# Patrick-McKeever/P2P-DHTs

Hardware: AMD Instinct MI355X
Metric: successor lookups/sec (whole node) + % HBM roofline, 2^24-peer ring, 1/2/4/8 GPUs (higher is better)
Workload: dtype u128; 1 GPU; C4 finger-routed lookups with hop counts (per GPU): 2^24-peer ring, 2^25 keys/GPU/step, src = q mod N, splitmix seeds 0x5EED0005/0x5EED0006; peers=16777216, keys_per_gpu=33554432, global_batch=33554432

## Files before the change

### p2p-dhts_amd/chordx/ring.py

```python
from __future__ import annotations

import ctypes

import numpy as np

from . import _lib as L

try:
    import torch
except Exception:
    torch = None


def _is_dev(x) -> bool:
    return torch is not None and isinstance(x, torch.Tensor) and x.is_cuda


def _keys_np(a) -> np.ndarray:
    return np.ascontiguousarray(np.asarray(a, dtype=np.uint64).reshape(-1, 2))


def _check_dev(t, esize: int, name: str, device=None, count=None):
    if not _is_dev(t):
        return
# ... 174 lines not shown
            sl = self._prep_u32(succs, "succs", self.n)
            ns = 1 if sl.ndim == 1 else int(sl.shape[1])
        arrs = [a for a in (al, sl) if a is not None]
        mk = self._mem(*arrs) if arrs else L.CX_MEM_HOST
        L.check(L.lib().cx_liveness_upload(self._h, _ptr(al), _ptr(sl), int(ns), int(rule), mk))

    def fingers_device(self):
        p = ctypes.c_void_p()
        L.check(L.lib().cx_fingers_device(self._h, ctypes.byref(p)))
        if not p.value:
            return None
        return _wrap_device(p.value, (self.n, L.CX_FINGERS), torch.int32, self.device, self)

    def set_route_variant(self, v: int):
        f = L.lib().cxi_set_route_variant
        f.argtypes = [ctypes.c_void_p, ctypes.c_int]
        L.check(f(self._h, v))

    def route_info(self):
        f = L.lib().cxi_route_info
        f.argtypes = [ctypes.c_void_p, ctypes.POINTER(ctypes.c_int),
                      ctypes.POINTER(ctypes.c_uint64), ctypes.POINTER(ctypes.c_uint64)]
        v, e, b = ctypes.c_int(), ctypes.c_uint64(), ctypes.c_uint64()
        L.check(f(self._h, ctypes.byref(v), ctypes.byref(e), ctypes.byref(b)))
        return v.value, e.value, b.value

    def route_counters(self, enable: bool):
        f = L.lib().cxi_route_counters
        f.argtypes = [ctypes.c_void_p, ctypes.c_int, ctypes.c_void_p]
        out = np.zeros(4, dtype=np.uint64)
        L.check(f(self._h, int(bool(enable)), _ptr(out)))
        return None if enable else tuple(int(x) for x in out)

    def gather_probe(self, lanes: int = 1 << 19, hops: int = 64, span: int = 0) -> float:
        if span:
            f = L.lib().cxi_gather_probe_span
            f.argtypes = [ctypes.c_void_p, ctypes.c_int, ctypes.c_int, ctypes.c_uint64,
                          ctypes.POINTER(ctypes.c_double)]
            r = ctypes.c_double()
            L.check(f(self._h, lanes, hops, span, ctypes.byref(r)))
            return r.value
        f = L.lib().cxi_gather_probe
        f.argtypes = [ctypes.c_void_p, ctypes.c_int, ctypes.c_int,
                      ctypes.POINTER(ctypes.c_double)]
        r = ctypes.c_double()
        L.check(f(self._h, lanes, hops, ctypes.byref(r)))
        return r.value

    def route_table_hash(self, arc: bool = False) -> int:
        f = L.lib().cxi_route_table_hash
        f.argtypes = [ctypes.c_void_p, ctypes.c_int, ctypes.POINTER(ctypes.c_uint64)]
        h = ctypes.c_uint64()
        L.check(f(self._h, int(bool(arc)), ctypes.byref(h)))
        return h.value

    def set_table_build(self, v: int):
        f = L.lib().cxi_set_table_build
        f.argtypes = [ctypes.c_void_p, ctypes.c_int]
        L.check(f(self._h, v))

    def set_route_depth(self, R: int):
        f = L.lib().cxi_set_route_depth
        f.argtypes = [ctypes.c_void_p, ctypes.c_int]
        L.check(f(self._h, int(R)))

    def set_fingers_repair(self, on: bool):
# ... 397 lines not shown
```

### p2p-dhts_amd/csrc/cx_api.hip

```cpp
#include <hip/hip_runtime.h>

#include <cstdio>
#include <cstdlib>
#include <cstring>
#include <initializer_list>
#include <algorithm>
#include <atomic>
#include <memory>
#include <mutex>
#include <string>
#include <vector>

#include "cx_kernels.hpp"

namespace {

thread_local std::string g_err;

int fail(int code, const std::string &msg) {
    g_err = msg;
    return code;
}

#define CX_HIP(expr)                                                                      \
// ... 311 lines not shown
    size_t n = 0;
    cell128 *d_ring = nullptr;
    size_t ring_cap = 0;
    cell128 *d_eyt = nullptr;
    uint32_t *d_fingers = nullptr;
    bool fingers_converged = false;
    std::atomic<bool> rows_deferred{false};
    std::mutex rows_mu;
    std::shared_ptr<PlaneSet> planes;
    std::shared_ptr<PlaneSet> parent_planes;
    int fingers_repair = 0;
    int planes_repaired = 0;
    uint64_t repair_searched = 0;
    cell128 *d_ring_ext = nullptr;
    int rt_l0 = 128, rt_R = 0;
    int depth_override = 0;
    uint64_t *d_tree = nullptr;
    bool tree_valid = false;
    int pk_ib = 1;
    uint64_t *d_cz = nullptr;
    int table_build = 0;
    bool cz_valid = false;
    uint64_t cz_escapes = 0;
    int route_variant = -1;
    cell128 *d_min_keys = nullptr;
    uint32_t *d_preds = nullptr;
    uint8_t *d_alive = nullptr;
    uint32_t *d_succs = nullptr;
    int succ_ns = 0;
    int fwd_rule = CX_FWD_CHORD;
    bool liveness = false;
    uint32_t *d_scratch = nullptr;
    unsigned long long *d_stats = nullptr;
    bool counting = false;
    uint64_t *d_arc_tree = nullptr;
    ArcBound *d_arc_bounds = nullptr;
    int arc_world = 0, arc_rank = -1, arc_Lh = 128, arc_nb = 0;
    uint32_t arc_plo = 0, arc_M = 0;
    size_t arc_bytes = 0;

    uint4 *d_dir = nullptr;
    uint32_t *d_ring_key = nullptr;
    int dir_k = 1;
    int search_variant = 1;
    void *d_sltab = nullptr;
    int sl_b = 0, sl_steps = 0;
    bool sl_dev16 = false;
    std::mutex sl_mu;
    std::atomic<bool> sl_ready{false};
    cell128 *d_stree = nullptr;
    uint32_t *d_eyt_rank = nullptr;
    int churn_variant = 1;
    uint64_t serial = 0;
    uint64_t churn_parent = 0;
    uint32_t *d_o2n_canon = nullptr;
    size_t o2n_canon_n = 0;
    uint4 *d_cdir = nullptr;
    int cdir_kb = 0;
    size_t cdir_bytes = 0;
    int misplaced_variant = 1;

    EytView eyt() const {
        EytView v;
        v.E = d_eyt;
        v.n = (uint32_t)n;
        v.h = 63 - __builtin_clzll((unsigned long long)n);
// ... 52 lines not shown
}

template <class T>
int stage_out(T *dst, size_t count, int memkind, DBuf &tmp, T **dev, hipStream_t s) {
    if (count == 0) {
        *dev = dst;
        return CX_OK;
    }
    CX_CHECK(dst != nullptr, CX_E_INVALID, "null output buffer");
    if (memkind == CX_MEM_DEVICE) {
        *dev = dst;
        return CX_OK;
    }
    CX_CHECK(memkind == CX_MEM_HOST, CX_E_INVALID, "bad memkind");
    CX_HIP(tmp.alloc_stage(count * sizeof(T), s));
    *dev = tmp.as<T>();
    return CX_OK;
}

template <class T>
int finish_out(T *dst, const T *dev, size_t count, int memkind, hipStream_t s) {
    if (memkind == CX_MEM_HOST && count) {
        CX_HIP(hipMemcpyAsync(dst, dev, count * sizeof(T), hipMemcpyDeviceToHost, s));
        CX_HIP(hipStreamSynchronize(s));
    }
    return CX_OK;
}

int sync_if_host(int memkind, hipStream_t s) {
    if (memkind == CX_MEM_HOST) CX_HIP(hipStreamSynchronize(s));
    return CX_OK;
}

struct RingRes {
    int device;
    hipStream_t stream;
    void *scratch;
};
std::mutex g_res_mu;
std::vector<RingRes> g_res;
constexpr size_t RES_KEEP = 16;

int alloc_ring(int device, cx_ring **out) {
    cx_ring *r = new cx_ring();
    r->device = device;
    {
        std::lock_guard<std::mutex> g(g_res_mu);
        for (size_t k = g_res.size(); k-- > 0;)
            if (g_res[k].device == device) {
                r->own_stream = g_res[k].stream;
                r->d_scratch = static_cast<uint32_t *>(g_res[k].scratch);
                g_res.erase(g_res.begin() + k);
                break;
            }
    }
    if (!r->own_stream) {
        hipError_t e = hipStreamCreateWithFlags(&r->own_stream, hipStreamNonBlocking);
        if (e != hipSuccess) {
            delete r;
            return fail(CX_E_HIP, std::string("hipStreamCreate: ") + hipGetErrorString(e));
        }
        e = dev_malloc(&r->d_scratch, 1024);
        if (e != hipSuccess) {
            (void)hipStreamDestroy(r->own_stream);
            delete r;
            return fail(CX_E_HIP, std::string("hipMalloc: ") + hipGetErrorString(e));
        }
    }
    r->stream = r->own_stream;
    static std::atomic<uint64_t> next_serial{1};
    r->serial = next_serial++;
    *out = r;
    return CX_OK;
}

void free_ring(cx_ring *r) {
    if (!r) return;
    (void)hipSetDevice(r->device);
    if (r->stream) (void)hipStreamSynchronize(r->stream);
    if (r->own_stream) (void)hipStreamSynchronize(r->own_stream);
    r->planes.reset();
    r->parent_planes.reset();
    table_free(r->device, r->d_ring, r->ring_cap * sizeof(cell128));
    (void)hipFree(r->d_eyt);
    table_free(r->device, r->d_dir, r->d_dir ? ((size_t)1 << r->dir_k) * sizeof(uint4) : 0);
    table_free(r->device, r->d_ring_key, r->n * sizeof(uint32_t));
    const size_t ent = r->n * (size_t)r->rt_R;
    table_free(r->device, r->d_fingers, r->n * CX_FINGERS * sizeof(uint32_t));
    table_free(r->device, r->d_tree, ent * 64);
    table_free(r->device, r->d_cz, ent * 128);
    (void)hipFree(r->d_stree);
    (void)hipFree(r->d_eyt_rank);
    (void)hipFree(r->d_sltab);
    table_free(r->device, r->d_ring_ext, (r->n + 1) * sizeof(cell128));
    (void)hipFree(r->d_min_keys);
    (void)hipFree(r->d_preds);
    (void)hipFree(r->d_alive);
    (void)hipFree(r->d_succs);
    table_free(r->device, r->d_arc_tree, r->arc_bytes);
// ... 807 lines not shown

int cx_route(const cx_ring *ring, const uint32_t *src, const cx_u128 *keys, size_t q,
             uint32_t *owner, uint8_t *hops, uint8_t *status, int memkind) {
    CX_CHECK(ring != nullptr, CX_E_INVALID, "null ring");
    CX_CHECK(ring->d_fingers != nullptr || ring->rows_deferred, CX_E_STATE,
             "finger table not built (cx_fingers_build / cx_fingers_upload)");
    int rc = use_device(ring);
    if (rc) return rc;
    hipStream_t s = ring->stream;
    DBuf ts, tk, to, th, tst;
    const uint32_t *dsrc;
    const cx_u128 *dk;
    uint32_t *dow;
    uint8_t *dh, *dst = nullptr;
    if ((rc = stage_in(src, q, memkind, ts, &dsrc, s))) return rc;
    if ((rc = stage_in(keys, q, memkind, tk, &dk, s))) return rc;
    if ((rc = stage_out(owner, q, memkind, to, &dow, s))) return rc;
    if ((rc = stage_out(hops, q, memkind, th, &dh, s))) return rc;
    if (status && (rc = stage_out(status, q, memkind, tst, &dst, s))) return rc;
    if (!ring->literal()) {
        int e2 = ensure_route_table(const_cast<cx_ring *>(ring), s);
        if (e2) return e2;
    }
    const int v = ring->literal() ? -1 : ring->variant();
    if (v != 5 || !ring->cz_valid) {
        int e2 = ensure_fingers_rows(const_cast<cx_ring *>(ring), s);
        if (e2) return e2;
    }
    SearchView dsv = ring->sv();
    dsv.dir = ring->d_dir;
    if (v == 5 && ring->cz_valid)
        CX_HIP(cxk::route_walk(ring->d_ring_ext, ring->d_ring, ring->n, ring->d_cz, ring->rt_l0,
                               ring->pk_ib, dsv, dsrc, reinterpret_cast<const cell128 *>(dk), q,
                               dow, dh, dst, ring->counting ? ring->d_stats : nullptr, s));
    else if (v == 4 && ring->tree_valid)
        CX_HIP(cxk::route_tree(ring->d_ring_ext, ring->d_ring, ring->n, ring->d_tree, ring->rt_l0,
                               ring->rt_R, ring->pk_ib, ring->d_fingers, dsrc,
                               reinterpret_cast<const cell128 *>(dk), q, dow, dh, dst, s));
    else
        CX_HIP(cxk::route(ring->d_ring, ring->n, ring->d_fingers, ring->d_min_keys,
                          ring->d_preds, ring->lit(), ring->literal(), dsrc,
                          reinterpret_cast<const cell128 *>(dk), q, dow, dh, dst, s));
    if (memkind == CX_MEM_HOST && q) {
        CX_HIP(hipMemcpyAsync(owner, dow, q * sizeof(uint32_t), hipMemcpyDeviceToHost, s));
        CX_HIP(hipMemcpyAsync(hops, dh, q, hipMemcpyDeviceToHost, s));
        if (status) CX_HIP(hipMemcpyAsync(status, dst, q, hipMemcpyDeviceToHost, s));
        CX_HIP(hipStreamSynchronize(s));
    }
    return CX_OK;
}

int cx_nsucc(const cx_ring *ring, const cx_u128 *keys, size_t q, int n, uint32_t *lists,
             uint8_t *count, int memkind) {
    CX_CHECK(ring != nullptr, CX_E_INVALID, "null ring");
    CX_CHECK(n >= 1 && n <= CX_MAX_NSUCC, CX_E_INVALID, "n must be in [1, 16]");
    int rc = use_device(ring);
    if (rc) return rc;
    hipStream_t s = ring->stream;
    DBuf tk, tl, tc;
    const cx_u128 *dk;
    uint32_t *dl;
    uint8_t *dc;
    if ((rc = stage_in(keys, q, memkind, tk, &dk, s))) return rc;
    if ((rc = stage_out(lists, q * (size_t)n, memkind, tl, &dl, s))) return rc;
    if ((rc = stage_out(count, q, memkind, tc, &dc, s))) return rc;
    CX_HIP(cxk::nsucc(ring->sv(), reinterpret_cast<const cell128 *>(dk), q, n, dl, dc, s));
    if (memkind == CX_MEM_HOST && q) {
// ... 982 lines not shown
    CX_CHECK(variant == -1 || variant == 0 || variant == 4 || variant == 5, CX_E_INVALID,
             "variant must be -1 (auto), 0, 4 or 5");
    ring->route_variant = variant;
    return CX_OK;
}

int cxi_set_route_depth(cx_ring *ring, int R) {
    CX_CHECK(ring != nullptr, CX_E_INVALID, "null ring");
    CX_CHECK(R == 0 || (R >= 16 && R <= 59), CX_E_INVALID, "R must be 0 or in [16, 59]");
    CX_CHECK(!ring->d_cz && !ring->d_tree && !ring->d_arc_tree,
             CX_E_STATE, "route depth is fixed once a route table exists");
    ring->depth_override = R;
    return CX_OK;
}

int cxi_route_info(const cx_ring *ring, int *variant, uint64_t *cz_escapes,
                   uint64_t *table_bytes) {
    CX_CHECK(ring && variant && cz_escapes && table_bytes, CX_E_INVALID, "null argument");
    const int v = ring->literal() ? -1 : ring->variant();
    const size_t ent = ring->n * (size_t)ring->rt_R;
    *variant = v;
    *cz_escapes = ring->cz_escapes;
    *table_bytes = v == 5 && ring->cz_valid     ? ent * 128
                   : v == 4 && ring->tree_valid ? ent * 64
                                                : 0;
    return CX_OK;
}

int cxi_route_counters(cx_ring *ring, int enable, uint64_t *out) {
    CX_CHECK(ring != nullptr, CX_E_INVALID, "null ring");
    int rc = use_device(ring);
    if (rc) return rc;
    hipStream_t s = ring->stream;
    if (!ring->d_stats) CX_HIP(dev_malloc(&ring->d_stats, 4 * sizeof(unsigned long long)));
    if (enable) {
        CX_HIP(hipMemsetAsync(ring->d_stats, 0, 4 * sizeof(unsigned long long), s));
        ring->counting = true;
        return CX_OK;
    }
    ring->counting = false;
    CX_CHECK(out != nullptr, CX_E_INVALID, "null out");
    unsigned long long h[4];
    CX_HIP(hipMemcpyAsync(h, ring->d_stats, sizeof(h), hipMemcpyDeviceToHost, s));
    CX_HIP(hipStreamSynchronize(s));
    for (int k = 0; k < 4; ++k) out[k] = h[k];
    return CX_OK;
}

int cxi_gather_probe(const cx_ring *ring, int lanes, int hops, double *rate) {
    CX_CHECK(ring && rate, CX_E_INVALID, "null argument");
    int rc = use_device(ring);
    if (rc) return rc;
    const void *t = nullptr;
    size_t bytes = 0;
    if (ring->cz_valid) {
        t = ring->d_cz;
        bytes = ring->n * (size_t)ring->rt_R * 128;
    } else if (ring->d_fingers) {
        t = ring->d_fingers;
        bytes = ring->n * (size_t)CX_FINGERS * sizeof(uint32_t);
    }
    CX_CHECK(t != nullptr, CX_E_STATE, "no route table built");
    CX_HIP(cxk::gather_probe(t, bytes, lanes, hops, rate, ring->stream));
    return CX_OK;
}

int cxi_gather_probe_span(const cx_ring *ring, int lanes, int hops, uint64_t span_bytes,
                          double *rate) {
    CX_CHECK(ring && rate, CX_E_INVALID, "null argument");
    CX_CHECK(ring->cz_valid, CX_E_STATE, "no pattern-keyed table built");
    int rc = use_device(ring);
    if (rc) return rc;
    size_t bytes = ring->n * (size_t)ring->rt_R * 128;
    if (span_bytes && span_bytes < bytes) bytes = span_bytes & ~(uint64_t)63;
    CX_CHECK(bytes >= 64 * 1024, CX_E_INVALID, "span too small");
    CX_HIP(cxk::gather_probe(ring->d_cz, bytes, lanes, hops, rate, ring->stream));
    return CX_OK;
}
// ... 138 lines not shown
```

### p2p-dhts_amd/csrc/cx_kernels.hpp

```cpp
#pragma once

#include "cx_common.hpp"

#define CX_TAG_JOIN 0x80000000u

struct alignas(16) ArcRec {
    uint64_t w0, w1;
    uint64_t qid;
    uint32_t cur;
    uint32_t hk;
};
static_assert(sizeof(ArcRec) == 32, "ArcRec is 32 B");
#define ARC_ORIGIN_SHIFT 40
struct ArcBound {
    uint64_t lo, hi;
    uint32_t rank, pad;
};
#define ARC_INDEX_MASK ((1ull << ARC_ORIGIN_SHIFT) - 1)
#define ARC_HINT_LOCAL 0xFFFFFFFFFFFFFFFFull
#define ARC_HINT_BAD 0xFFFFFFFFFFFFFFFEull
enum { ARC_NEW = 0, ARC_RESULT = 1, ARC_WALK = 2, ARC_NONE = 3 };

#define IDA_GUARD_WORD 0xA5C3A5C3u
#define IDA_GUARD_WORDS 64
// ... 85 lines not shown
    static FingerView planes(const uint32_t *FT, size_t n, int L, int nl) {
        return FingerView{FT, 1, n, L, nl, nullptr, 0};
    }
};
hipError_t table_hash(const void *t, size_t bytes, unsigned long long *out, hipStream_t s);
#define CX_STREE_MAX 10
struct STreeView {
    const cell128 *lv[CX_STREE_MAX];
    uint32_t sz[CX_STREE_MAX];
    int top;
    size_t words;
    int lds_from;
    uint32_t lds_off[CX_STREE_MAX];
};
STreeView stree_plan(const cell128 *ring, size_t n, cell128 *buf);
hipError_t stree_build(const STreeView &v, hipStream_t s);
hipError_t successor_stree(const STreeView &st, const cell128 *keys, size_t q, uint32_t *owner,
                           bool pred, hipStream_t s);
hipError_t eyt_rank_build(size_t n, uint32_t *rank, hipStream_t s);
hipError_t successor_eyt16(const EytView &ev, const uint32_t *rank, const cell128 *keys, size_t q,
                           uint32_t *owner, bool pred, hipStream_t s);
hipError_t fingers_levels(const uint32_t *F, size_t n, int L, int nl, uint32_t *FT,
                          hipStream_t s);
hipError_t fingers_pairs(const uint32_t *FT, size_t n, int nl, uint32_t *C2, hipStream_t s);
hipError_t ring_hi(const cell128 *ring, size_t n, uint64_t *hi, hipStream_t s);
hipError_t ring_codes(const cell128 *ring, size_t n, int ib, uint32_t *rs, uint32_t *wide,
                      hipStream_t s);
hipError_t cz_build(const FingerView &fv, const cell128 *ring, const uint64_t *rh, size_t n,
                    int l0, int R, int ib, uint64_t *cz, uint32_t *esc, hipStream_t s,
                    uint32_t *ws = nullptr);
size_t cz_build_ws_words(size_t n, int lvl_base, int nlev, uint32_t M);
uint32_t cz2_cap();
void cz2_set_cap(uint32_t cap);
hipError_t route_walk(const cell128 *ring_ext, const cell128 *ring, size_t n, const uint64_t *cz,
                      int l0, int ib, const SearchView &sv, const uint32_t *src,
                      const cell128 *keys, size_t q, uint32_t *owner, uint8_t *hops,
                      uint8_t *status, unsigned long long *stats, hipStream_t s);
hipError_t gather_probe(const void *table, size_t bytes, int lanes, int hops, double *rate,
                        hipStream_t s);
hipError_t cz_build_part(const FingerView &fv, const cell128 *ring, const uint64_t *rh, size_t n,
                         int lvl_base, int nlev, uint32_t p_first, uint32_t M, int ib,
                         uint64_t *cz, uint32_t *esc, hipStream_t s, uint32_t *ws = nullptr);
hipError_t route_arc(const cell128 *ring_ext, const cell128 *ring, size_t n, const uint64_t *cz,
                     int l0, int R, int ib, const SearchView &sv, int Lh, uint32_t plo, uint32_t M,
                     int self, const ArcRec *in, const uint32_t *src, const cell128 *keys, size_t q,
                     ArcRec *out, uint32_t *owner, uint8_t *hops, uint8_t *status, hipStream_t s);
hipError_t route_walk_arc(const cell128 *ring_ext, const cell128 *ring, size_t n,
                          const uint64_t *arc_tree, int l0, int ib, const SearchView &sv, int Lh,
                          uint32_t plo, uint32_t M, const uint32_t *src, const cell128 *keys,
                          size_t q, const uint64_t *dh, uint64_t *res, hipStream_t s);
hipError_t route_walk_arc_local(const cell128 *ring_ext, const cell128 *ring, size_t n,
                                const uint64_t *arc_tree, int l0, int ib, const SearchView &sv,
                                int Lh, uint32_t plo, uint32_t M, const uint32_t *src,
                                const cell128 *keys, const uint32_t *idx, size_t q,
                                uint32_t *owner, uint8_t *hops, uint8_t *status, hipStream_t s);
hipError_t arc_partition(const uint32_t *src, const cell128 *keys, size_t q,
                         const ArcBound *bounds, int nb, int G, uint32_t *counts_dev,
                         uint32_t *cursor_dev, cell128 *skeys, uint32_t *ssrc, uint32_t *perm,
                         hipStream_t s);
hipError_t arc_partition_regions(const uint32_t *src, const cell128 *keys, size_t q,
                                 const ArcBound *bounds, int nb, int G, uint32_t cap,
                                 uint32_t *cursor_dev, uint32_t *ovf, cell128 *skeys,
                                 uint32_t *ssrc, uint32_t *perm, uint64_t *sd,
                                 const cell128 *ring_ext, size_t n, int ib, hipStream_t s);
hipError_t arc_count_keys(const cell128 *keys, size_t q, const ArcBound *bounds, int nb, int G,
                          int64_t *counts, int me, uint32_t *own_idx, uint32_t *own_ws,
                          hipStream_t s);
hipError_t arc_scatter_exact(const uint32_t *src, const cell128 *keys, size_t q,
                             const ArcBound *bounds, int nb, int G, const int64_t *counts,
                             uint32_t *cursor, cell128 *skeys, uint32_t *ssrc, uint32_t *perm,
// ... 74 lines not shown
```

### p2p-dhts_amd/csrc/cx_walk.hip

```cpp
#include "cx_kernels.hpp"

namespace cxk {
namespace {

constexpr int WK_BLOCK = 256;
constexpr uint32_t WK_NONE = 0xFFFFFFFFu;
constexpr uint32_t WK_CZ_NONE = 0xFFFFFFFFu;
constexpr uint32_t CX_QI_ARC_MISS = 0xFE;

enum { M_NONE = 0, M_HOP = 1, M_FIX = 2, M_EXACT = 3, M_FIXT = 4 };
enum { B_EMPTY = 0, B_KEYS = 1, B_READY = 2, B_IDX = 3 };
enum { P_WALK = 0, P_LOCAL = 1, P_BAD = 2 };

struct WalkIO {
    const cell128 *ring_ext;
    const cell128 *ring;
    uint32_t n;
    const uint4 *cz;
    int l0, gs;
    SearchView sv;
    const uint32_t *src;
    const cell128 *keys;
    size_t q, chunk;
    uint32_t *owner;
    uint8_t *hops, *status;
    unsigned long long *stats;
    int Lh;
    uint32_t plo, M;
    const uint64_t *dh;
    uint64_t *res_out;
    const uint32_t *idx;
};

__device__ __forceinline__ uint32_t wk_expect(uint32_t n, int l) {
    const int sh = 128 - l;
    return sh >= 32 ? 0u : (n + (1u << (sh - 1))) >> sh;
}

__device__ __forceinline__ uint32_t wk_next(const uint32_t *Etab, uint32_t n, uint32_t cur, int l,
                                            uint32_t wd) {
    const uint32_t t = cur + Etab[l] + (wd & 0xFFFFu);
    return min(t, min(t + n, t - n));
}

__device__ __forceinline__ uint64_t wk_units(u128 x, int gs) {
    return (uint64_t)(x >> 64) >> (gs - 64);
}

__device__ __forceinline__ u128 wk_u128(const unsigned int __attribute__((ext_vector_type(4))) v) {
    return ((u128)(((uint64_t)v.w << 32) | v.z) << 64) | (((uint64_t)v.y << 32) | v.x);
}

__device__ __forceinline__ uint64_t wk_pack(uint32_t own, uint32_t h, uint32_t st) {
    return (1ull << 63) | ((uint64_t)st << 40) | ((uint64_t)(h & 0xFF) << 32) | own;
}

#ifdef CX_WALK_WPE
#define WK_ATTR __attribute__((amdgpu_waves_per_eu(CX_WALK_WPE)))
#else
#define WK_ATTR
#endif

template <bool STATS, bool KF, bool IX = false>
__global__ __launch_bounds__(WK_BLOCK) WK_ATTR void k_walk(WalkIO io) {
    constexpr bool PACK = KF && !IX;
    constexpr int RG = 260;
    __shared__ uint32_t ent_all[WK_BLOCK / 64][4 * RG];
    __shared__ uint32_t Etab[CX_FINGERS];
    const uint32_t n = io.n;
    for (int l = threadIdx.x; l < (int)CX_FINGERS; l += WK_BLOCK) Etab[l] = wk_expect(n, l) - 32768u;
    __syncthreads();
    const int l0 = io.l0, gs = io.gs;
    const int lane = threadIdx.x & 63, qs = threadIdx.x & 3;
    uint32_t *ent_w = ent_all[threadIdx.x >> 6];
    const uint32_t *ent = ent_w + (lane & 3) * RG + (lane >> 2) * 16;
    const size_t wave = __builtin_amdgcn_readfirstlane(
        (uint32_t)((blockIdx.x * (size_t)WK_BLOCK + threadIdx.x) >> 6));
    const size_t base = wave * io.chunk;
    if (base >= io.q) return;
    const uint32_t cnt = (uint32_t)((base + io.chunk < io.q) ? io.chunk : io.q - base);
    const size_t ab = IX ? 0 : base;
    uint32_t *const own_w = PACK ? nullptr : io.owner + ab;
    uint8_t *const hop_w = PACK ? nullptr : io.hops + ab;
    uint8_t *const st_w = PACK || !io.status ? nullptr : io.status + ab;
    uint64_t *const res_w = PACK ? io.res_out + base : nullptr;
    const cell128 *const key_r = io.keys + ab;
    const uint32_t *const src_r = io.src + ab;
    const uint64_t *const dh_r = PACK && io.dh ? io.dh + base : nullptr;
    const uint32_t *const idx_r = IX ? io.idx + base : nullptr;
    auto put = [&](uint32_t o, uint32_t ow, uint32_t hh, uint32_t st) {
        if (PACK) {
            res_w[o] = wk_pack(ow, hh, st);
        } else {
            own_w[o] = ow;
            hop_w[o] = (uint8_t)hh;
            if (st_w) st_w[o] = (uint8_t)st;
        }
    };
    uint32_t head = 0;

    int mode = M_NONE, lvl = 0, rb = 0;
    uint32_t cur = 0, h = 0, pn = 0;
    uint64_t dmin = 0, dmax = 0;
    u128 key = 0;
    uint32_t qi = 0;
    int bst = B_EMPTY, pst = P_WALK;
    uint32_t pq = 0;
    u128 pkey = 0;
    uint32_t psrc = 0;
    uint64_t pd = 0;
    uint32_t n_g64 = 0, n_r16 = 0, n_xc = 0, n_q = 0;
    const uint32_t arc_top = KF ? (uint32_t)(CX_FINGERS - io.Lh) * 2u * n : 0u;

    for (;;) {
        if (__ballot(mode != M_NONE || bst != B_EMPTY) == 0 && head >= cnt)
            break;

        uint32_t eidx = WK_NONE;
        if (mode == M_HOP) {
            if (!KF)
                eidx = (uint32_t)((lvl - l0) * 2 + rb) * n + cur;
            else if (lvl >= io.Lh)
                eidx = (uint32_t)((lvl - io.Lh) * 2 + rb) * n + cur;
            else
                eidx = arc_top + (uint32_t)((lvl - l0) * 2 + rb) * io.M +
                       (cur >= io.plo ? cur - io.plo : cur + n - io.plo);
        }
        if (STATS) {
            n_g64 += mode == M_HOP;
            n_r16 += mode == M_FIX ? 1u : (mode >= M_EXACT ? 2u : 0u);
        }
        typedef unsigned int v4n __attribute__((ext_vector_type(4)));
        const bool pair_now = bst == B_KEYS;
        v4n pa4 = {0, 0, 0, 0}, pb4 = {0, 0, 0, 0};
        if ((!PACK || !io.dh) && pair_now && psrc < n) {
            pa4 = __builtin_nontemporal_load(reinterpret_cast<const v4n *>(io.ring_ext + psrc));
            pb4 = __builtin_nontemporal_load(reinterpret_cast<const v4n *>(io.ring_ext + psrc + 1));
        }
        if (IX && bst == B_IDX) {
            pkey = ld128(key_r + pq);
            psrc = src_r[pq];
            bst = B_KEYS;
        }
        {
            const uint32_t avail = cnt - head;
            const uint64_t want = __ballot(bst == B_EMPTY);
            const uint32_t rank = __builtin_amdgcn_mbcnt_hi(
                (uint32_t)(want >> 32), __builtin_amdgcn_mbcnt_lo((uint32_t)want, 0u));
            if (bst == B_EMPTY && rank < avail) {
                if (IX) {
                    pq = idx_r[head + rank];
                    bst = B_IDX;
                } else {
                    pq = head + rank;
                    pkey = ld128(key_r + pq);
                    psrc = src_r[pq];
                    if (PACK && io.dh) pd = dh_r[pq];
                    bst = B_KEYS;
                }
            }
            const uint32_t took = (uint32_t)__popcll(want);
            head += took < avail ? took : avail;
        }
        const uint32_t ek[4] = {(uint32_t)__builtin_amdgcn_mov_dpp((int)eidx, 0x00, 0xF, 0xF, false),
                                (uint32_t)__builtin_amdgcn_mov_dpp((int)eidx, 0x55, 0xF, 0xF, false),
                                (uint32_t)__builtin_amdgcn_mov_dpp((int)eidx, 0xAA, 0xF, 0xF, false),
                                (uint32_t)__builtin_amdgcn_mov_dpp((int)eidx, 0xFF, 0xF, 0xF, false)};
#pragma unroll
        for (int k = 0; k < 4; ++k)
            if (ek[k] != WK_NONE)
                __builtin_amdgcn_global_load_lds(
                    (const __attribute__((address_space(1))) void *)(io.cz + (size_t)ek[k] * 4 + qs),
                    (__attribute__((address_space(3))) void *)(ent_w + k * RG), 16, 0, 2 );
        v4n xa4 = {0, 0, 0, 0}, xb4 = {0, 0, 0, 0};
        if (mode >= M_FIX) {
            xa4 = *reinterpret_cast<const v4n *>(io.ring + cur);
            if (mode != M_FIX)
                xb4 = *reinterpret_cast<const v4n *>(io.ring + (mode == M_FIXT ? pn : (cur + 1 == n ? 0u : cur + 1)));
        }
        asm volatile("s_waitcnt vmcnt(0)" ::: "memory");
        __builtin_amdgcn_fence(__ATOMIC_RELEASE, "wavefront");
        __builtin_amdgcn_wave_barrier();
        __builtin_amdgcn_fence(__ATOMIC_ACQUIRE, "wavefront");
        asm volatile("" : "+v"(pa4), "+v"(pb4), "+v"(xa4), "+v"(xb4));
        const u128 pa = wk_u128(pa4), pb = wk_u128(pb4), xa = wk_u128(xa4), xb = wk_u128(xb4);

        if (PACK && io.dh && pair_now) {
            pst = psrc >= n || pd == ARC_HINT_BAD ? P_BAD : (pd == ARC_HINT_LOCAL ? P_LOCAL : P_WALK);
            bst = B_READY;
        } else if (pair_now) {
            if (psrc >= n) {
                pst = P_BAD;
            } else if (n == 1 || (pkey - pa - 1) <= (pb - pa - 1)) {
                pst = P_LOCAL;
            } else {
                pst = P_WALK;
                pd = wk_units(pkey - pb, gs);
            }
            bst = B_READY;
        }

        uint32_t own = CX_NONE, st = CX_Q_OK;
        bool fin = false, plan = false;
        if (mode >= M_FIX) {
            const u128 d = key - xa;
            if (mode == M_FIX) {
                dmin = dmax = wk_units(d, gs);
                plan = true;
            } else if (mode == M_FIXT) {
                if (d <= xb - xa) {
                    fin = true;
                    own = pn;
                } else {
                    cur = pn;
                    dmin = dmax = wk_units(key - xb, gs);
                    plan = true;
                }
// ... 56 lines not shown
            bool vv;
            if (o == 1) {
                v = 0;
                vv = cs == 16;
            } else {
                v = (cs & 15) | (1 << (o - 2));
                vv = cs < 16 && !(rb && v == 15);
            }
            const uint32_t wd = ent[v];
            const bool ok = need && vv && dmin >= T && wd != WK_CZ_NONE;
            const uint64_t e = T + (wd >> 16);
            const uint32_t nxt = wk_next(Etab, n, cur, l, wd);
            const bool own_now = ok && dmax < e;
            const bool und = ok && !own_now && dmin <= e;
            const bool mv = ok && !own_now && !und;
            h += ok ? 1u : 0u;
            if (own_now) own = nxt;
            fin = fin || own_now;
            if (und) {
                pn = nxt;
                mode = M_FIXT;
            }
            cur = mv ? nxt : cur;
            dmin = mv ? dmin - e - 1 : dmin;
            dmax = mv ? dmax - e : dmax;
            cs = mv ? v : ((need || !act) ? -1 : cs);
        }
        if (mode == M_HOP && !fin) plan = true;

        if (fin) {
            put(qi, own, h, st);
            mode = M_NONE;
        }
        if (!plan && mode == M_NONE && bst == B_READY) {
            bst = B_EMPTY;
            qi = pq;
            key = pkey;
            cur = psrc;
            h = 0;
            if (STATS) ++n_q;
            if (pst == P_WALK) {
                dmin = dmax = pd;
                plan = true;
            } else {
                put(qi, pst == P_LOCAL ? cur : CX_NONE, 0, pst == P_LOCAL ? CX_Q_OK : CX_Q_BADPEER);
            }
        }

        if (plan) {
            if (dmin == 0) {
                mode = M_EXACT;
            } else {
                const int ma = 63 - __builtin_clzll(dmin), mb = 63 - __builtin_clzll(dmax);
                if (ma != mb) {
                    mode = M_FIX;
                } else if (ma + gs >= l0) {
                    mode = M_HOP;
                    lvl = ma + gs;
                    rb = ma >= 1 ? (int)((dmax >> (ma - 1)) & 1) : 0;
                    if (KF && lvl < io.Lh && (cur >= io.plo ? cur - io.plo : cur + n - io.plo) >= io.M) {
                        mode = M_NONE;
                        put(qi, CX_NONE, h, CX_QI_ARC_MISS);
                    }
                } else {
                    mode = M_EXACT;
                }
            }
        }
    }
    if (STATS) {
        uint64_t v[4] = {n_g64, n_r16, n_xc, n_q};
#pragma unroll
        for (int k = 0; k < 4; ++k) {
#pragma unroll
            for (int off = 32; off > 0; off >>= 1) v[k] += __shfl_xor(v[k], off, 64);
        }
        if (lane == 0)
#pragma unroll
            for (int k = 0; k < 4; ++k) atomicAdd(io.stats + k, (unsigned long long)v[k]);
    }
}

constexpr size_t WK_MIN_PER_WAVE = 64;
#ifndef CX_WALK_WAVES
#define CX_WALK_WAVES 7
#endif

template <class K>
size_t walk_lds_pad(K kernel) {
    hipFuncAttributes fa{};
    if (hipFuncGetAttributes(&fa, reinterpret_cast<const void *>(kernel)) != hipSuccess) return 0;
    const size_t lds = 160 * 1024, cap = lds / (CX_WALK_WAVES + 1) + 256;
    return fa.sharedSizeBytes < cap ? cap - fa.sharedSizeBytes : 0;
}

template <class K>
unsigned walk_resident_grid(K kernel, size_t pad) {
    int dev = 0, cus = 256, per = 1;
    (void)hipGetDevice(&dev);
    (void)hipDeviceGetAttribute(&cus, hipDeviceAttributeMultiprocessorCount, dev);
    if (hipOccupancyMaxActiveBlocksPerMultiprocessor(&per, kernel, WK_BLOCK, pad) != hipSuccess ||
        per < 1)
        per = 1;
    return (unsigned)(per * cus);
}

}

hipError_t route_walk(const cell128 *ring_ext, const cell128 *ring, size_t n, const uint64_t *cz,
                      int l0, int ib, const SearchView &sv, const uint32_t *src,
                      const cell128 *keys, size_t q, uint32_t *owner, uint8_t *hops,
                      uint8_t *status, unsigned long long *stats, hipStream_t s) {
    if (q == 0) return hipSuccess;
    const int gs = cz_shift(ib);
    if (n == 0 || n >= (1u << 30) || gs < 64 || l0 < 5 || (size_t)(128 - l0) * 2 * n >= WK_NONE)
        return hipErrorInvalidValue;
    WalkIO io = {};
    io.ring_ext = ring_ext;
    io.ring = ring;
    io.n = (uint32_t)n;
    io.cz = reinterpret_cast<const uint4 *>(cz);
    io.l0 = l0;
    io.gs = gs;
    io.sv = sv;
    io.src = src;
    io.keys = keys;
    io.q = q;
    io.owner = owner;
    io.hops = hops;
    io.status = status;
    io.stats = stats;
    static const size_t pad = walk_lds_pad(k_walk<false, false>);
    static const unsigned resident = walk_resident_grid(k_walk<false, false>, pad);
    size_t waves = (size_t)resident * (WK_BLOCK / 64);
    const size_t small = (q + WK_MIN_PER_WAVE - 1) / WK_MIN_PER_WAVE;
    if (small < waves) waves = small ? small : 1;
    io.chunk = (q + waves - 1) / waves;
    if (io.chunk >= (1ull << 32)) return hipErrorInvalidValue;
    waves = (q + io.chunk - 1) / io.chunk;
    const unsigned blocks = (unsigned)((waves * 64 + WK_BLOCK - 1) / WK_BLOCK);
    if (stats)
        k_walk<true, false><<<blocks, WK_BLOCK, pad, s>>>(io);
    else
        k_walk<false, false><<<blocks, WK_BLOCK, pad, s>>>(io);
    return hipGetLastError();
}

hipError_t route_walk_arc(const cell128 *ring_ext, const cell128 *ring, size_t n,
                          const uint64_t *arc_tree, int l0, int ib, const SearchView &sv, int Lh,
                          uint32_t plo, uint32_t M, const uint32_t *src, const cell128 *keys,
                          size_t q, const uint64_t *dh, uint64_t *res, hipStream_t s) {
    if (q == 0) return hipSuccess;
    const int gs = cz_shift(ib);
    if (n == 0 || n >= (1u << 30) || gs < 64 || l0 < 5 || Lh < l0 || Lh > (int)CX_FINGERS ||
        M > n || (size_t)(CX_FINGERS - Lh) * 2 * n + (size_t)(Lh - l0) * 2 * M >= WK_NONE)
        return hipErrorInvalidValue;
    WalkIO io = {};
    io.ring_ext = ring_ext;
    io.ring = ring;
    io.n = (uint32_t)n;
    io.cz = reinterpret_cast<const uint4 *>(arc_tree);
    io.l0 = l0;
    io.gs = gs;
    io.sv = sv;
    io.src = src;
    io.keys = keys;
    io.q = q;
    io.Lh = Lh;
    io.plo = plo;
    io.M = M;
    io.dh = dh;
    io.res_out = res;
    static const size_t pad = walk_lds_pad(k_walk<false, true>);
    static const unsigned resident = walk_resident_grid(k_walk<false, true>, pad);
    size_t waves = (size_t)resident * (WK_BLOCK / 64);
    const size_t small = (q + WK_MIN_PER_WAVE - 1) / WK_MIN_PER_WAVE;
    if (small < waves) waves = small ? small : 1;
    io.chunk = (q + waves - 1) / waves;
// ... 50 lines not shown
```

Measured before the change: 10.75 billion lookups/s.

## Add dynamic work-claiming and LDS key staging to the route walk kernel

Replaces the static per-wave chunking of lookups in the walk kernel with a global atomic claim counter, so waves grab 32-512-lookup blocks on demand and load imbalance from variable hop counts is reduced. Keys and sources are also staged into LDS via global_load_lds in batches of 32, instead of being loaded per lane. A per-ring rotating claim slot is reset by the last finishing wave, and per-wave timestamp stats plus Python probes are added. It adds atomic traffic, extra LDS use and a waves_per_eu attribute change that may alter occupancy.

Measured after the change: 10.42 billion lookups/s. 0.969x the previous value.

```diff
diff --git a/p2p-dhts_amd/chordx/ring.py b/p2p-dhts_amd/chordx/ring.py
--- a/p2p-dhts_amd/chordx/ring.py
+++ b/p2p-dhts_amd/chordx/ring.py
@@ -230,6 +230,25 @@
         L.check(f(self._h, int(bool(enable)), _ptr(out)))
         return None if enable else tuple(int(x) for x in out)
 
+    def route_wave_times(self):
+        f = L.lib().cxi_route_wave_times
+        f.argtypes = [ctypes.c_void_p, ctypes.c_void_p, ctypes.c_size_t]
+        out = np.zeros(4 + 16384, dtype=np.uint64)
+        L.check(f(self._h, _ptr(out), out.size))
+        return int(out[0]), int(out[2]), out[4:4 + min(int(out[1]), 16384)].copy()
+
+    def route_walk_shape(self, q: int):
+        f = L.lib().cxi_route_walk_shape
+        f.argtypes = [ctypes.c_void_p, ctypes.c_size_t, ctypes.c_void_p]
+        out = np.zeros(4, dtype=np.uint64)
+        L.check(f(self._h, int(q), _ptr(out)))
+        return tuple(int(x) for x in out)
+
+    def set_walk_claim_min(self, lookups_per_wave: int):
+        f = L.lib().cxi_route_claim_min
+        f.argtypes = [ctypes.c_void_p, ctypes.c_size_t]
+        L.check(f(self._h, int(lookups_per_wave)))
+
     def gather_probe(self, lanes: int = 1 << 19, hops: int = 64, span: int = 0) -> float:
         if span:
             f = L.lib().cxi_gather_probe_span
diff --git a/p2p-dhts_amd/csrc/cx_api.hip b/p2p-dhts_amd/csrc/cx_api.hip
--- a/p2p-dhts_amd/csrc/cx_api.hip
+++ b/p2p-dhts_amd/csrc/cx_api.hip
@@ -367,6 +367,8 @@
     bool liveness = false;
     uint32_t *d_scratch = nullptr;
     unsigned long long *d_stats = nullptr;
+    mutable std::atomic<uint32_t> walk_seq{0};
+    size_t walk_claim_min = 0;
     bool counting = false;
     uint64_t *d_arc_tree = nullptr;
     ArcBound *d_arc_bounds = nullptr;
@@ -485,6 +487,8 @@
     return CX_OK;
 }
 
+constexpr size_t SCRATCH_WORDS = 256, SCRATCH_WALK_CLAIM = 256, SCRATCH_WALK_SLOTS = 128;
+constexpr size_t SCRATCH_BYTES = (SCRATCH_WORDS + 2 * SCRATCH_WALK_SLOTS) * sizeof(uint32_t);
 struct RingRes {
     int device;
     hipStream_t stream;
@@ -513,11 +517,20 @@
             delete r;
             return fail(CX_E_HIP, std::string("hipStreamCreate: ") + hipGetErrorString(e));
         }
-        e = dev_malloc(&r->d_scratch, 1024);
+        e = dev_malloc(&r->d_scratch, SCRATCH_BYTES);
         if (e != hipSuccess) {
             (void)hipStreamDestroy(r->own_stream);
             delete r;
             return fail(CX_E_HIP, std::string("hipMalloc: ") + hipGetErrorString(e));
+        }
+        e = hipMemsetAsync(r->d_scratch + SCRATCH_WALK_CLAIM, 0,
+                           2 * SCRATCH_WALK_SLOTS * sizeof(uint32_t), r->own_stream);
+        if (e == hipSuccess) e = hipStreamSynchronize(r->own_stream);
+        if (e != hipSuccess) {
+            (void)hipStreamDestroy(r->own_stream);
+            (void)hipFree(r->d_scratch);
+            delete r;
+            return fail(CX_E_HIP, std::string("hipMemset: ") + hipGetErrorString(e));
         }
     }
     r->stream = r->own_stream;
@@ -1391,7 +1404,10 @@
     if (v == 5 && ring->cz_valid)
         CX_HIP(cxk::route_walk(ring->d_ring_ext, ring->d_ring, ring->n, ring->d_cz, ring->rt_l0,
                                ring->pk_ib, dsv, dsrc, reinterpret_cast<const cell128 *>(dk), q,
-                               dow, dh, dst, ring->counting ? ring->d_stats : nullptr, s));
+                               dow, dh, dst, ring->counting ? ring->d_stats : nullptr,
+                               ring->d_scratch + SCRATCH_WALK_CLAIM +
+                                   2 * (ring->walk_seq++ % SCRATCH_WALK_SLOTS),
+                               ring->walk_claim_min, s));
     else if (v == 4 && ring->tree_valid)
         CX_HIP(cxk::route_tree(ring->d_ring_ext, ring->d_ring, ring->n, ring->d_tree, ring->rt_l0,
                                ring->rt_R, ring->pk_ib, ring->d_fingers, dsrc,
@@ -2440,9 +2456,11 @@
     int rc = use_device(ring);
     if (rc) return rc;
     hipStream_t s = ring->stream;
-    if (!ring->d_stats) CX_HIP(dev_malloc(&ring->d_stats, 4 * sizeof(unsigned long long)));
+    if (!ring->d_stats)
+        CX_HIP(dev_malloc(&ring->d_stats, cxk::WK_STAT_WORDS * sizeof(unsigned long long)));
     if (enable) {
-        CX_HIP(hipMemsetAsync(ring->d_stats, 0, 4 * sizeof(unsigned long long), s));
+        CX_HIP(hipMemsetAsync(ring->d_stats, 0, cxk::WK_STAT_WORDS * sizeof(unsigned long long), s));
+        CX_HIP(hipMemsetAsync(ring->d_stats + cxk::WK_STAT_START, 0xFF, sizeof(unsigned long long), s));
         ring->counting = true;
         return CX_OK;
     }
@@ -2452,6 +2470,36 @@
     CX_HIP(hipMemcpyAsync(h, ring->d_stats, sizeof(h), hipMemcpyDeviceToHost, s));
     CX_HIP(hipStreamSynchronize(s));
     for (int k = 0; k < 4; ++k) out[k] = h[k];
+    return CX_OK;
+}
+
+int cxi_route_wave_times(cx_ring *ring, uint64_t *out, size_t cap) {
+    CX_CHECK(ring && out && cap >= 4, CX_E_INVALID, "null argument");
+    CX_CHECK(ring->d_stats != nullptr, CX_E_STATE, "counters not enabled (cxi_route_counters)");
+    int rc = use_device(ring);
+    if (rc) return rc;
+    hipStream_t s = ring->stream;
+    const size_t w = std::min(cap - 4, (size_t)cxk::WK_STAT_WAVES);
+    CX_HIP(hipMemcpyAsync(out, ring->d_stats + cxk::WK_STAT_START, 4 * sizeof(uint64_t),
+                          hipMemcpyDeviceToHost, s));
+    if (w)
+        CX_HIP(hipMemcpyAsync(out + 4, ring->d_stats + cxk::WK_STAT_END, w * sizeof(uint64_t),
+                              hipMemcpyDeviceToHost, s));
+    CX_HIP(hipStreamSynchronize(s));
+    return CX_OK;
+}
+
+int cxi_route_walk_shape(const cx_ring *ring, size_t q, uint64_t *out) {
+    CX_CHECK(ring && out, CX_E_INVALID, "null argument");
+    int rc = use_device(ring);
+    if (rc) return rc;
+    cxk::route_walk_shape(q, true, ring->walk_claim_min, out);
+    return CX_OK;
+}
+
+int cxi_route_claim_min(cx_ring *ring, size_t lookups_per_wave) {
+    CX_CHECK(ring != nullptr, CX_E_INVALID, "null ring");
+    ring->walk_claim_min = lookups_per_wave;
     return CX_OK;
 }
 
diff --git a/p2p-dhts_amd/csrc/cx_kernels.hpp b/p2p-dhts_amd/csrc/cx_kernels.hpp
--- a/p2p-dhts_amd/csrc/cx_kernels.hpp
+++ b/p2p-dhts_amd/csrc/cx_kernels.hpp
@@ -141,10 +141,14 @@
 size_t cz_build_ws_words(size_t n, int lvl_base, int nlev, uint32_t M);
 uint32_t cz2_cap();
 void cz2_set_cap(uint32_t cap);
+constexpr size_t WK_STAT_START = 4, WK_STAT_END = 8, WK_STAT_WAVES = 16384;
+constexpr size_t WK_STAT_WORDS = WK_STAT_END + WK_STAT_WAVES;
 hipError_t route_walk(const cell128 *ring_ext, const cell128 *ring, size_t n, const uint64_t *cz,
                       int l0, int ib, const SearchView &sv, const uint32_t *src,
                       const cell128 *keys, size_t q, uint32_t *owner, uint8_t *hops,
-                      uint8_t *status, unsigned long long *stats, hipStream_t s);
+                      uint8_t *status, unsigned long long *stats, uint32_t *claim,
+                      size_t claim_min, hipStream_t s);
+void route_walk_shape(size_t q, bool claim, size_t claim_min, uint64_t out[4]);
 hipError_t gather_probe(const void *table, size_t bytes, int lanes, int hops, double *rate,
                         hipStream_t s);
 hipError_t cz_build_part(const FingerView &fv, const cell128 *ring, const uint64_t *rh, size_t n,
diff --git a/p2p-dhts_amd/csrc/cx_walk.hip b/p2p-dhts_amd/csrc/cx_walk.hip
--- a/p2p-dhts_amd/csrc/cx_walk.hip
+++ b/p2p-dhts_amd/csrc/cx_walk.hip
@@ -1,3 +1,5 @@
+#include <algorithm>
+
 #include "cx_kernels.hpp"
 
 namespace cxk {
@@ -30,7 +32,20 @@
     const uint64_t *dh;
     uint64_t *res_out;
     const uint32_t *idx;
+    uint32_t *claim;
+    uint32_t cu;
+    bool stage;
 };
+
+#ifndef WK_CLAIM
+#define WK_CLAIM 512
+#endif
+static_assert(WK_CLAIM % 32 == 0, "claims are whole 32-lookup blocks");
+constexpr size_t WK_CLAIM_MIN = 4 * (size_t)WK_CLAIM;
+#ifndef WK_STAGE
+#define WK_STAGE 1
+#endif
+constexpr uint32_t WK_STG = 32;
 
 __device__ __forceinline__ uint32_t wk_expect(uint32_t n, int l) {
     const int sh = 128 - l;
@@ -55,18 +70,25 @@
     return (1ull << 63) | ((uint64_t)st << 40) | ((uint64_t)(h & 0xFF) << 32) | own;
 }
 
+#ifndef CX_WALK_WAVES
+#define CX_WALK_WAVES 7
+#endif
 #ifdef CX_WALK_WPE
 #define WK_ATTR __attribute__((amdgpu_waves_per_eu(CX_WALK_WPE)))
 #else
-#define WK_ATTR
+#define WK_ATTR __attribute__((amdgpu_waves_per_eu(STATS ? CX_WALK_WAVES : 1)))
 #endif
 
 template <bool STATS, bool KF, bool IX = false>
 __global__ __launch_bounds__(WK_BLOCK) WK_ATTR void k_walk(WalkIO io) {
     constexpr bool PACK = KF && !IX;
+    constexpr bool CL = !KF;
+    constexpr bool CLM = CL && WK_CLAIM > 0;
+    constexpr bool ST = CL && WK_STAGE;
     constexpr int RG = 260;
     __shared__ uint32_t ent_all[WK_BLOCK / 64][4 * RG];
     __shared__ uint32_t Etab[CX_FINGERS];
+    __shared__ __attribute__((aligned(16))) uint32_t stg_all[WK_BLOCK / 64][5 * WK_STG];
     const uint32_t n = io.n;
     for (int l = threadIdx.x; l < (int)CX_FINGERS; l += WK_BLOCK) Etab[l] = wk_expect(n, l) - 32768u;
     __syncthreads();
@@ -74,12 +96,17 @@
     const int lane = threadIdx.x & 63, qs = threadIdx.x & 3;
     uint32_t *ent_w = ent_all[threadIdx.x >> 6];
     const uint32_t *ent = ent_w + (lane & 3) * RG + (lane >> 2) * 16;
+    uint32_t *stg_w = stg_all[threadIdx.x >> 6];
     const size_t wave = __builtin_amdgcn_readfirstlane(
         (uint32_t)((blockIdx.x * (size_t)WK_BLOCK + threadIdx.x) >> 6));
-    const size_t base = wave * io.chunk;
-    if (base >= io.q) return;
-    const uint32_t cnt = (uint32_t)((base + io.chunk < io.q) ? io.chunk : io.q - base);
-    const size_t ab = IX ? 0 : base;
+    if (STATS && lane == 0) atomicMin(io.stats + WK_STAT_START, (unsigned long long)wall_clock64());
+    bool more = CLM && io.claim != nullptr;
+    const size_t nwaves = (size_t)gridDim.x * (WK_BLOCK / 64);
+    const size_t base = wave * (more ? (size_t)io.cu : io.chunk);
+    if (!more && base >= io.q) return;
+    const size_t csz = more ? (size_t)io.cu : io.chunk;
+    const uint32_t cnt = base >= io.q ? 0u : (uint32_t)((base + csz < io.q) ? csz : io.q - base);
+    const size_t ab = IX || CL ? 0 : base;
     uint32_t *const own_w = PACK ? nullptr : io.owner + ab;
     uint8_t *const hop_w = PACK ? nullptr : io.hops + ab;
     uint8_t *const st_w = PACK || !io.status ? nullptr : io.status + ab;
@@ -97,7 +124,10 @@
             if (st_w) st_w[o] = (uint8_t)st;
         }
     };
-    uint32_t head = 0;
+    uint32_t head = CL && cnt ? (uint32_t)base : 0u, end = head + cnt, nb = 0;
+    bool has_nb = false;
+    const bool staged = ST && io.stage;
+    uint32_t sb = 0, sn = 0, sc = 0;
 
     int mode = M_NONE, lvl = 0, rb = 0;
     uint32_t cur = 0, h = 0, pn = 0;
@@ -109,11 +139,18 @@
     u128 pkey = 0;
     uint32_t psrc = 0;
     uint64_t pd = 0;
-    uint32_t n_g64 = 0, n_r16 = 0, n_xc = 0, n_q = 0;
+    uint32_t n_xc = 0;
+    unsigned long long n_g64 = 0, n_r16 = 0, n_q = 0;
     const uint32_t arc_top = KF ? (uint32_t)(CX_FINGERS - io.Lh) * 2u * n : 0u;
 
     for (;;) {
-        if (__ballot(mode != M_NONE || bst != B_EMPTY) == 0 && head >= cnt)
+        if (CLM && head >= end && has_nb) {
+            head = nb;
+            end = (uint32_t)((size_t)nb + io.cu < io.q ? (size_t)nb + io.cu : io.q);
+            has_nb = false;
+        }
+        if (__ballot(mode != M_NONE || bst != B_EMPTY) == 0 && head >= end && !more &&
+            (!ST || sc >= sn))
             break;
 
         uint32_t eidx = WK_NONE;
@@ -127,8 +164,8 @@
                        (cur >= io.plo ? cur - io.plo : cur + n - io.plo);
         }
         if (STATS) {
-            n_g64 += mode == M_HOP;
-            n_r16 += mode == M_FIX ? 1u : (mode >= M_EXACT ? 2u : 0u);
+            n_g64 += __popcll(__ballot(mode == M_HOP));
+            n_r16 += __popcll(__ballot(mode == M_FIX)) + 2 * __popcll(__ballot(mode >= M_EXACT));
         }
         typedef unsigned int v4n __attribute__((ext_vector_type(4)));
         const bool pair_now = bst == B_KEYS;
@@ -142,8 +179,12 @@
             psrc = src_r[pq];
             bst = B_KEYS;
         }
+        const bool claim_now = CLM && more && !has_nb && end - head < 64;
+        uint32_t ck = 0;
+        if (CLM && claim_now && lane == 0)
+            ck = __hip_atomic_fetch_add(io.claim, 1u, __ATOMIC_RELAXED, __HIP_MEMORY_SCOPE_AGENT);
         {
-            const uint32_t avail = cnt - head;
+            const uint32_t avail = ST && staged ? sn - sc : end - head;
             const uint64_t want = __ballot(bst == B_EMPTY);
             const uint32_t rank = __builtin_amdgcn_mbcnt_hi(
                 (uint32_t)(want >> 32), __builtin_amdgcn_mbcnt_lo((uint32_t)want, 0u));
@@ -151,6 +192,12 @@
                 if (IX) {
                     pq = idx_r[head + rank];
                     bst = B_IDX;
+                } else if (ST && staged) {
+                    const uint32_t o = sc + rank;
+                    pq = sb + o;
+                    pkey = wk_u128(*reinterpret_cast<const v4n *>(stg_w + 4 * o));
+                    psrc = stg_w[4 * WK_STG + o];
+                    bst = B_KEYS;
                 } else {
                     pq = head + rank;
                     pkey = ld128(key_r + pq);
@@ -160,7 +207,10 @@
                 }
             }
             const uint32_t took = (uint32_t)__popcll(want);
-            head += took < avail ? took : avail;
+            if (ST && staged)
+                sc += took < avail ? took : avail;
+            else
+                head += took < avail ? took : avail;
         }
         const uint32_t ek[4] = {(uint32_t)__builtin_amdgcn_mov_dpp((int)eidx, 0x00, 0xF, 0xF, false),
                                 (uint32_t)__builtin_amdgcn_mov_dpp((int)eidx, 0x55, 0xF, 0xF, false),
@@ -178,11 +228,37 @@
             if (mode != M_FIX)
                 xb4 = *reinterpret_cast<const v4n *>(io.ring + (mode == M_FIXT ? pn : (cur + 1 == n ? 0u : cur + 1)));
         }
+        if (ST && staged && sc >= sn && head < end) {
+            asm volatile("s_waitcnt lgkmcnt(0)" ::: "memory");
+            const uint32_t m = end - head < WK_STG ? end - head : WK_STG;
+            if ((uint32_t)lane < m) {
+                __builtin_amdgcn_global_load_lds(
+                    (const __attribute__((address_space(1))) void *)(io.keys + head + lane),
+                    (__attribute__((address_space(3))) void *)stg_w, 16, 0, 2 );
+                __builtin_amdgcn_global_load_lds(
+                    (const __attribute__((address_space(1))) void *)(io.src + head + lane),
+                    (__attribute__((address_space(3))) void *)(stg_w + 4 * WK_STG), 4, 0, 2 );
+            }
+            sb = head;
+            sn = m;
+            sc = 0;
+            head += m;
+        }
         asm volatile("s_waitcnt vmcnt(0)" ::: "memory");
         __builtin_amdgcn_fence(__ATOMIC_RELEASE, "wavefront");
         __builtin_amdgcn_wave_barrier();
         __builtin_amdgcn_fence(__ATOMIC_ACQUIRE, "wavefront");
         asm volatile("" : "+v"(pa4), "+v"(pb4), "+v"(xa4), "+v"(xb4));
+        if (CLM && claim_now) {
+            asm volatile("" : "+v"(ck));
+            const size_t b = (nwaves + __builtin_amdgcn_readfirstlane(ck)) * (size_t)io.cu;
+            if (b < io.q) {
+                nb = (uint32_t)b;
+                has_nb = true;
+            } else {
+                more = false;
+            }
+        }
         const u128 pa = wk_u128(pa4), pb = wk_u128(pb4), xa = wk_u128(xa4), xb = wk_u128(xb4);
 
         if (PACK && io.dh && pair_now) {
@@ -305,13 +381,13 @@
             put(qi, own, h, st);
             mode = M_NONE;
         }
+        if (STATS) n_q += __popcll(__ballot(!plan && mode == M_NONE && bst == B_READY));
         if (!plan && mode == M_NONE && bst == B_READY) {
             bst = B_EMPTY;
             qi = pq;
             key = pkey;
             cur = psrc;
             h = 0;
-            if (STATS) ++n_q;
             if (pst == P_WALK) {
                 dmin = dmax = pd;
                 plan = true;
@@ -341,29 +417,42 @@
             }
         }
     }
+    if (CLM && io.claim != nullptr && lane == 0) {
+        const uint32_t done =
+            __hip_atomic_fetch_add(io.claim + 1, 1u, __ATOMIC_RELAXED, __HIP_MEMORY_SCOPE_AGENT);
+        if (done + 1 == (uint32_t)nwaves) {
+            __hip_atomic_exchange(io.claim, 0u, __ATOMIC_RELAXED, __HIP_MEMORY_SCOPE_AGENT);
+            __hip_atomic_exchange(io.claim + 1, 0u, __ATOMIC_RELAXED, __HIP_MEMORY_SCOPE_AGENT);
+        }
+    }
     if (STATS) {
-        uint64_t v[4] = {n_g64, n_r16, n_xc, n_q};
+        if (lane == 0) {
+            if (wave < WK_STAT_WAVES) io.stats[WK_STAT_END + wave] = wall_clock64();
+            if (wave == 0) {
+                io.stats[WK_STAT_START + 1] = nwaves;
+                io.stats[WK_STAT_START + 2] = CLM && io.claim ? io.cu : 0;
+            }
+        }
+        uint64_t xc = n_xc;
 #pragma unroll
-        for (int k = 0; k < 4; ++k) {
-#pragma unroll
-            for (int off = 32; off > 0; off >>= 1) v[k] += __shfl_xor(v[k], off, 64);
-        }
+        for (int off = 32; off > 0; off >>= 1) xc += __shfl_xor(xc, off, 64);
+        const unsigned long long v[4] = {n_g64, n_r16, xc, n_q};
         if (lane == 0)
 #pragma unroll
-            for (int k = 0; k < 4; ++k) atomicAdd(io.stats + k, (unsigned long long)v[k]);
+            for (int k = 0; k < 4; ++k) atomicAdd(io.stats + k, v[k]);
     }
 }
 
 constexpr size_t WK_MIN_PER_WAVE = 64;
-#ifndef CX_WALK_WAVES
-#define CX_WALK_WAVES 7
-#endif
+
+constexpr size_t WK_NO_PAD = ~(size_t)0;
 
 template <class K>
 size_t walk_lds_pad(K kernel) {
     hipFuncAttributes fa{};
     if (hipFuncGetAttributes(&fa, reinterpret_cast<const void *>(kernel)) != hipSuccess) return 0;
     const size_t lds = 160 * 1024, cap = lds / (CX_WALK_WAVES + 1) + 256;
+    if (fa.sharedSizeBytes > lds / CX_WALK_WAVES) return WK_NO_PAD;
     return fa.sharedSizeBytes < cap ? cap - fa.sharedSizeBytes : 0;
 }
 
@@ -378,13 +467,57 @@
     return (unsigned)(per * cus);
 }
 
+struct WalkShape {
+    size_t pad, resident, chunk;
+    unsigned blocks;
+    uint32_t cu;
+    bool stage;
+};
+
+WalkShape walk_shape(size_t q, bool claim, size_t claim_min) {
+    static const size_t pad = walk_lds_pad(k_walk<false, false>);
+    static const unsigned resident =
+        walk_resident_grid(k_walk<false, false>, pad == WK_NO_PAD ? 0 : pad);
+    WalkShape sh = {};
+    sh.pad = pad;
+    size_t waves = (size_t)resident * (WK_BLOCK / 64);
+    sh.resident = waves;
+    const size_t small = (q + WK_MIN_PER_WAVE - 1) / WK_MIN_PER_WAVE;
+    if (WK_CLAIM > 0 && claim && small >= waves &&
+        q / waves >= (claim_min ? claim_min : WK_CLAIM_MIN)) {
+        sh.stage = WK_STAGE;
+        const size_t quarter = (q / waves / 4) & ~(size_t)31;
+        sh.cu = (uint32_t)std::min<size_t>(WK_CLAIM, std::max<size_t>(32, quarter));
+        sh.chunk = sh.cu;
+        sh.blocks = resident;
+        return sh;
+    }
+    if (small < waves) waves = small ? small : 1;
+    sh.chunk = (q + waves - 1) / waves;
+    waves = (q + sh.chunk - 1) / sh.chunk;
+    sh.blocks = (unsigned)((waves * 64 + WK_BLOCK - 1) / WK_BLOCK);
+    return sh;
+}
+
 }
 
 hipError_t route_walk(const cell128 *ring_ext, const cell128 *ring, size_t n, const uint64_t *cz,
                       int l0, int ib, const SearchView &sv, const uint32_t *src,
                       const cell128 *keys, size_t q, uint32_t *owner, uint8_t *hops,
-                      uint8_t *status, unsigned long long *stats, hipStream_t s) {
+                      uint8_t *status, unsigned long long *stats, uint32_t *claim,
+                      size_t claim_min, hipStream_t s) {
     if (q == 0) return hipSuccess;
+    constexpr size_t slice = (size_t)1 << 31;
+    if (q >= 2 * slice) {
+        for (size_t o = 0; o < q; o += slice) {
+            const hipError_t e =
+                route_walk(ring_ext, ring, n, cz, l0, ib, sv, src + o, keys + o,
+                           std::min(slice, q - o), owner + o, hops + o,
+                           status ? status + o : nullptr, stats, claim, claim_min, s);
+            if (e != hipSuccess) return e;
+        }
+        return hipSuccess;
+    }
     const int gs = cz_shift(ib);
     if (n == 0 || n >= (1u << 30) || gs < 64 || l0 < 5 || (size_t)(128 - l0) * 2 * n >= WK_NONE)
         return hipErrorInvalidValue;
@@ -403,20 +536,25 @@
     io.hops = hops;
     io.status = status;
     io.stats = stats;
-    static const size_t pad = walk_lds_pad(k_walk<false, false>);
-    static const unsigned resident = walk_resident_grid(k_walk<false, false>, pad);
-    size_t waves = (size_t)resident * (WK_BLOCK / 64);
-    const size_t small = (q + WK_MIN_PER_WAVE - 1) / WK_MIN_PER_WAVE;
-    if (small < waves) waves = small ? small : 1;
-    io.chunk = (q + waves - 1) / waves;
-    if (io.chunk >= (1ull << 32)) return hipErrorInvalidValue;
-    waves = (q + io.chunk - 1) / io.chunk;
-    const unsigned blocks = (unsigned)((waves * 64 + WK_BLOCK - 1) / WK_BLOCK);
+    const WalkShape sh = walk_shape(q, claim != nullptr, claim_min);
+    if (sh.pad == WK_NO_PAD) return hipErrorInvalidConfiguration;
+    io.chunk = sh.chunk;
+    io.stage = sh.stage;
+    io.claim = sh.cu ? claim : nullptr;
+    io.cu = sh.cu;
     if (stats)
-        k_walk<true, false><<<blocks, WK_BLOCK, pad, s>>>(io);
+        k_walk<true, false><<<sh.blocks, WK_BLOCK, sh.pad, s>>>(io);
     else
-        k_walk<false, false><<<blocks, WK_BLOCK, pad, s>>>(io);
+        k_walk<false, false><<<sh.blocks, WK_BLOCK, sh.pad, s>>>(io);
     return hipGetLastError();
+}
+
+void route_walk_shape(size_t q, bool claim, size_t claim_min, uint64_t out[4]) {
+    const WalkShape sh = walk_shape(q, claim, claim_min);
+    out[0] = sh.resident;
+    out[1] = (uint64_t)sh.blocks * (WK_BLOCK / 64);
+    out[2] = sh.cu;
+    out[3] = WK_CLAIM;
 }
 
 hipError_t route_walk_arc(const cell128 *ring_ext, const cell128 *ring, size_t n,
```
